# jcasal-homer/HomerHEVC

Hardware: AMD Instinct MI355X
Metric: encoded frames/sec, 1080p & 2160p YUV420 fixed-QP IPPP, 1/2/4/8 MI355X (higher is better)
Workload: dtype int16; 1 GPU; cfg2-1080p-encode; sequences_per_gpu=256, width=1920, height=1080, wfpp_num_threads=17, qp=32, gop=IPPP intra_period=100

## Files before the change

homerhevc_amd/csrc/enc/enc_common.h:

```cpp
#pragma once
#include "enc_prims.h"
#if !defined(__HIPCC__)
#include <stdio.h>
#include <stdlib.h>
#endif

#if !defined(__HIPCC__) && defined(HENC_TRACE_ENABLE)
#include <stdio.h>
extern "C" FILE *henc_trace_file;
#define HENC_TRACE(...) do { if (henc_trace_file) fprintf(henc_trace_file, __VA_ARGS__); } while (0)
#define HENC_TRACE_PW(e, tag)                                                                                                                      \
	do {                                                                                                                                       \
		if (henc_trace_file) {                                                                                                             \
			unsigned a_[3] = {0, 0, 0};                                                                                                \
			for (int c_ = 0; c_ < 3; c_++) {                                                                                           \
				const int n_ = c_ ? 32 : 64;                                                                                       \
				const pred_t *p_ = c_ ? (e).w->pred_c[c_ - 1] : (e).w->pred_y;                                                     \
				for (int y_ = 0; y_ < n_; y_++)                                                                                    \
					for (int x_ = 0; x_ < n_; x_++) a_[c_] += (unsigned)(p_[y_ * n_ + x_] & 0xffff) * (unsigned)(1 + ((x_ + 3 * y_) & 7)); \
			}                                                                                                                          \
			fprintf(henc_trace_file, "PW %s ctu=%d pred=%u,%u,%u\n", tag, (e).ctu->ctu_number, a_[0], a_[1], a_[2]);                   \
		}                                                                                                                                  \
	} while (0)
#else
// ... 324 lines not shown
	HENC_ENC_IN_LDS(e);
	const Geo &gq = e.geo[ni];
	*idx = gq.abs_top_left;
	if (gq.raster_index == 0) return ctu_top_left_of(e);
	if (gq.raster_index < 16) return ctu_top_of(e);
	if ((gq.raster_index & 15) == 0) return ctu_left_of(e);
	return e.ctu;
}

template <class G>
HENC_HD void sync_reference_buffs(const G g, Enc &__restrict__ e, int ni, int src_wnd, int dst_wnd)
{
	HENC_ENC_IN_LDS(e);
	PRIM_T0();
	const Geo &q = e.geo[ni];
	const int16_t *s = dec_ptr(*e.w, src_wnd, COMP_Y) + q.y * DEC_STRIDE_Y + q.x;
	int16_t *d = dec_ptr(*e.w, dst_wnd, COMP_Y) + q.y * DEC_STRIDE_Y + q.x;
	const int n = q.size;
	for (int i = g.tid; i < 2 * n - 1; i += g.n) {
		const int off = i < n ? (n - 1) * DEC_STRIDE_Y + i : (i - n) * DEC_STRIDE_Y + n - 1;
		d[off] = s[off];
	}
	g.sync();
	PRIM_END(PP_SYNC);
}
template <class G>
HENC_HD void sync_reference_buffs_range(const G g, Enc &__restrict__ e, int ni, int src_wnd, int first_dst, int last_dst)
{
	HENC_ENC_IN_LDS(e);
	PRIM_T0();
	const Geo &q = e.geo[ni];
	const int16_t *s = dec_ptr(*e.w, src_wnd, COMP_Y) + q.y * DEC_STRIDE_Y + q.x;
	const int n = q.size, base = q.y * DEC_STRIDE_Y + q.x;
	for (int i0 = g.tid; i0 < 2 * n - 1; i0 += 2 * g.n) {
		const int i1 = i0 + g.n;
		const int off0 = i0 < n ? (n - 1) * DEC_STRIDE_Y + i0 : (i0 - n) * DEC_STRIDE_Y + n - 1;
		const int off1 = i1 < n ? (n - 1) * DEC_STRIDE_Y + i1 : (i1 - n) * DEC_STRIDE_Y + n - 1;
		const bool two = i1 < 2 * n - 1;
		const int16_t v0 = s[off0], v1 = two ? s[off1] : (int16_t)0;
		for (int wnd = first_dst; wnd <= last_dst; wnd++) {
			int16_t *d = dec_ptr(*e.w, wnd, COMP_Y) + base;
			d[off0] = v0;
			if (two) d[off1] = v1;
		}
	}
	g.sync();
	PRIM_END(PP_SYNC);
}
template <class G>
HENC_HD void sync_reference_buffs_chroma(const G g, Enc &__restrict__ e, int ni, int src_wnd, int dst_wnd)
{
	HENC_ENC_IN_LDS(e);
	PRIM_T0();
	const Geo &q = e.geo[ni];
	const int n = q.size_chroma;
	const int16_t *su = dec_ptr(*e.w, src_wnd, COMP_U) + q.yc * DEC_STRIDE_C + q.xc, *sv = dec_ptr(*e.w, src_wnd, COMP_V) + q.yc * DEC_STRIDE_C + q.xc;
	int16_t *du = dec_ptr(*e.w, dst_wnd, COMP_U) + q.yc * DEC_STRIDE_C + q.xc, *dv = dec_ptr(*e.w, dst_wnd, COMP_V) + q.yc * DEC_STRIDE_C + q.xc;
	for (int i = g.tid; i < 2 * n - 1; i += g.n) {
		const int off = i < n ? (n - 1) * DEC_STRIDE_C + i : (i - n) * DEC_STRIDE_C + n - 1;
		const int16_t a = su[off], b = sv[off];
		du[off] = a;
		dv[off] = b;
	}
	g.sync();
	PRIM_END(PP_SYNC);
}
template <class G>
HENC_HD void sync_cu_comp(const G g, Enc &__restrict__ e, int ni, int q_src, int q_dst, int d_src, int d_dst, int comp)
{
	HENC_ENC_IN_LDS(e);
	PRIM_T0();
	const Geo &q = e.geo[ni];
	const int n = comp == COMP_Y ? q.size : q.size_chroma, x = comp == COMP_Y ? q.x : q.xc, y = comp == COMP_Y ? q.y : q.yc;
	const int st = dec_stride(comp), off = comp == COMP_Y ? (q.abs_index << 4) : ((q.abs_index << 4) >> 2);
	const int16_t *ds = dec_ptr(*e.w, d_src, comp) + y * st + x;
	int16_t *dd = dec_ptr(*e.w, d_dst, comp) + y * st + x;
	const int16_t *qs = tq_ptr(*e.w, q_src, comp) + off;
	int16_t *qd = tq_ptr(*e.w, q_dst, comp) + off;
	const int ln = ilog2i(n);
	constexpr int BATCH = 4;
	for (int i0 = g.tid * 4; i0 < n * n; i0 += g.n * 4 * BATCH) {
		S4 a[BATCH], b[BATCH];
#pragma unroll
		for (int u = 0; u < BATCH; u++) {
			const int i = i0 + u * g.n * 4;
			if (i < n * n) {
				a[u] = ld4(ds + (i >> ln) * st + (i & (n - 1)));
				b[u] = ld4(qs + i);
			}
		}
#pragma unroll
		for (int u = 0; u < BATCH; u++) {
			const int i = i0 + u * g.n * 4;
			if (i < n * n) {
				st4(dd + (i >> ln) * st + (i & (n - 1)), a[u]);
				st4(qd + i, b[u]);
			}
		}
	}
	g.sync();
	PRIM_END(PP_SYNC);
}
template <class G>
HENC_HD void sync_cu_chroma_both(const G g, Enc &__restrict__ e, int ni, int q_src, int q_dst, int d_src, int d_dst)
{
	HENC_ENC_IN_LDS(e);
	PRIM_T0();
	const Geo &q = e.geo[ni];
	const int n = q.size_chroma, st = DEC_STRIDE_C, off = (q.abs_index << 4) >> 2, ln = ilog2i(n);
	const int16_t *ds[2], *qs[2];
	int16_t *dd[2], *qd[2];
	for (int c = 0; c < 2; c++) {
		ds[c] = dec_ptr(*e.w, d_src, COMP_U + c) + q.yc * st + q.xc;
		dd[c] = dec_ptr(*e.w, d_dst, COMP_U + c) + q.yc * st + q.xc;
		qs[c] = tq_ptr(*e.w, q_src, COMP_U + c) + off;
		qd[c] = tq_ptr(*e.w, q_dst, COMP_U + c) + off;
	}
	constexpr int BATCH = 2;
	for (int i0 = g.tid * 4; i0 < n * n; i0 += g.n * 4 * BATCH) {
		S4 a[2][BATCH], b[2][BATCH];
#pragma unroll
		for (int u = 0; u < BATCH; u++) {
			const int i = i0 + u * g.n * 4;
			if (i < n * n)
				for (int c = 0; c < 2; c++) {
					a[c][u] = ld4(ds[c] + (i >> ln) * st + (i & (n - 1)));
					b[c][u] = ld4(qs[c] + i);
				}
		}
#pragma unroll
		for (int u = 0; u < BATCH; u++) {
			const int i = i0 + u * g.n * 4;
			if (i < n * n)
				for (int c = 0; c < 2; c++) {
					st4(dd[c] + (i >> ln) * st + (i & (n - 1)), a[c][u]);
					st4(qd[c] + i, b[c][u]);
				}
		}
	}
	g.sync();
	PRIM_END(PP_SYNC);
}
template <class G>
HENC_HD void sync_motion_buffers_luma(const G g, Enc &__restrict__ e, int ni, int q_src, int q_dst, int d_src, int d_dst)
{
	HENC_ENC_IN_LDS(e);
	sync_cu_comp(g, e, ni, q_src, q_dst, d_src, d_dst, COMP_Y);
}
template <class G>
HENC_HD void sync_motion_buffers_chroma(const G g, Enc &__restrict__ e, int ni, int q_src, int q_dst, int d_src, int d_dst)
// ... 62 lines not shown
```

homerhevc_amd/csrc/enc/enc_ctu.h:

```cpp
#pragma once
#include "enc_intra.h"
#include "enc_inter.h"
#include "enc_quad.h"

namespace henc {

template <class G>
HENC_HD void info_buffs_copy(const G g, Enc &__restrict__ e, int depth, int abs_idx, int num, int to_ctu)
{
	HENC_ENC_IN_LDS(e);
	PRIM_T0();
	Work &w = *e.w;
	CtuPublic &c = *e.ctu;
	for (int i = g.tid; i < num; i += g.n) {
		const int k = abs_idx + i;
		if (to_ctu) {
			c.cbf[0][k] = w.cbf_buffs[0][depth][k];
			c.cbf[1][k] = w.cbf_buffs[1][depth][k];
			c.cbf[2][k] = w.cbf_buffs[2][depth][k];
			c.tr_idx[k] = w.tr_idx_buffs[depth][k];
			c.intra_mode[0][k] = w.intra_mode_buffs[0][depth][k];
			c.intra_mode[1][k] = w.intra_mode_buffs[1][depth][k];
		} else {
			const uint8_t v0 = c.cbf[0][k], v1 = c.cbf[1][k], v2 = c.cbf[2][k], v3 = c.tr_idx[k], v4 = c.intra_mode[0][k], v5 = c.intra_mode[1][k];
// ... 738 lines not shown
		blk_copy_to_src(g, e.f->src[comp] + py * ss + px, ss, curr_ptr(w, comp), sz, hh, ww);
	}
	if (c.has_left || c.has_top) {
		for (int comp = 0; comp < 3; comp++) {
			const int sz = comp ? 32 : 64, px = comp ? c.x >> 1 : c.x, py = comp ? c.y >> 1 : c.y;
			const int pw = comp ? S.width >> 1 : S.width, ph = comp ? S.height >> 1 : S.height;
			const int rs = comp ? S.stride_c : S.stride_y, ds = dec_stride(comp);
			int left_copy = 0, top_copy = 0;
			if (c.has_left) left_copy += sz;
			if (c.has_top) top_copy += sz;
			if (c.has_top_right) top_copy += sz;
			if (left_copy > ph - py) left_copy = ph - py;
			if (top_copy > pw - px) top_copy = pw - px;
			const int16_t *src = e.f->rec[comp] + py * rs + px;
			for (int l = 0; l < NWND; l++) {
				int16_t *dst = dec_ptr(w, l, comp);
				for (int i = g.tid; i < 1 + top_copy + left_copy; i += g.n) {
					if (i == 0) {
						if (c.has_left && c.has_top) dst[-ds - 1] = src[-rs - 1];
					} else if (i <= top_copy) dst[-ds + (i - 1)] = src[-rs + (i - 1)];
					else {
						const int j = i - 1 - top_copy;
						dst[j * ds - 1] = src[j * rs - 1];
					}
				}
			}
		}
		g.sync();
	}
	create_partition_neighbours(g, e);
	if (HENC_HELPERS(e)) {
// ... 70 lines not shown
```

homerhevc_amd/csrc/enc/enc_inter.h:

```cpp
#pragma once
#include "enc_common.h"

namespace henc {

#if !defined(__HIPCC__)
template <class G>
HENC_HD void mc_luma_interp(const G g, Enc &__restrict__ e, const int16_t *ref, int rs, int16_t *pred, int ps, int n, int mvx, int mvy)
{
	HENC_ENC_IN_LDS(e);
	const int xf = mvx & 3, yf = mvy & 3;
	const int16_t *src = ref + (mvy >> 2) * rs + (mvx >> 2);
	if (xf == 0) interp_stage<8>(g, src, rs, pred, ps, yf, n, n, 1, 1, 1);
	else if (yf == 0) interp_stage<8>(g, src, rs, pred, ps, xf, n, n, 0, 1, 1);
	else {
		int16_t *tmp = e.mc_tmp_y;
		const int ts = e.mc_tmp_y_stride;
		interp_stage<8>(g, src - 3 * rs, rs, tmp, ts, xf, n, n + 7, 0, 1, 0);
		interp_stage<8>(g, tmp + 3 * ts, ts, pred, ps, yf, n, n, 1, 0, 1);
	}
}
template <class G>
HENC_HD void mc_chroma_interp(const G g, Enc &__restrict__ e, const int16_t *ref, int rs, int16_t *pred, int ps, int n, int mvx, int mvy)
{
	HENC_ENC_IN_LDS(e);
// ... 464 lines not shown
	const int original_depth = e.geo[ni].depth;
	const int pi = (comp == COMP_Y || e.geo[ni].size_chroma != 2) ? ni : e.geo[ni].parent;
	const Geo &q = e.geo[pi];
	const int is_y = comp == COMP_Y;
	const int curr_depth = q.depth, n = is_y ? q.size : q.size_chroma, x = is_y ? q.x : q.xc, y = is_y ? q.y : q.yc;
	const int cs = ctu_stride(comp), ds = dec_stride(comp);
	const int wnd = original_depth + 1 + (part_size_type != PART_2Nx2N);
	const int qp = is_y ? (int)nd.qp : chroma_qp_table((int)nd.qp + e.seq->chroma_qp_offset);
	const int per = qp / 6, rem = qp % 6;
	const double weight = is_y ? 1.0 : e.f->chroma_weight;
	const int off = is_y ? (q.abs_index << 4) : ((q.abs_index << 4) >> 2);
	const pred_t *pred = pred_ptr(w, comp) + y * cs + x;
	const src_t *orig = curr_ptr(w, comp) + y * cs + x;
	int16_t *quant = tq_ptr(w, wnd, comp) + off, *iquant = iq_slot(w, comp, off, e.on_helper) + scratch_off;
	int16_t *const scratch_a = e.scratch_a + scratch_off, *const scratch_b = e.scratch_b + scratch_off;
	int16_t *dec = dec_ptr(w, wnd, comp) + y * ds + x;
	int16_t *rdec = scratch_b;
	tr_forward(g, HENC_FT(e), e.T, orig, cs, pred, cs, scratch_a, scratch_b, n, 0);
	int sum = quantize(g, HENC_FT(e), e.T, scratch_a, iquant, scratch_b, SCAN_DIAG, curr_depth, comp, 0, e.f->slice_type == SLICE_I, e.seq->sign_hiding, n, per, rem);
	nd.inter_cbf[comp] = (sum ? 1 : 0) << (original_depth - depth);
	if (is_y) nd.inter_tr_idx = original_depth - depth;
	uint32_t ssd;
	const bool coded = sum > 0;
	uint32_t raw_zero = 0;
	if (coded) {
		lin_copy_nosync(g, iquant, quant, n * n);
		raw_zero = blk_ssd(g, orig, cs, pred, cs, n);
		if (raw_ssq) *raw_ssq = raw_zero;
		dequantize(g, HENC_FT(e), e.T, iquant, iquant, curr_depth, comp, 0, n, per, rem);
	}
#if defined(HENC_MFMA_TRANSFORM) && !defined(HENC_MFMA_NO_PAIR)
// ... 324 lines not shown
```

homerhevc_amd/csrc/enc/enc_intra.h:

```cpp
#pragma once
#include "enc_common.h"
#include "enc_rdo.h"

namespace henc {

HENC_INLINE int intra_is_filtered(int mode, int inv_depth)
{
	static constexpr int intra_filter[5] = {10, 7, 1, 0, 10};
	const int diff = hmin(habs(mode - HOR_IDX), habs(mode - VER_IDX));
	return (mode != DC_IDX) && (diff > intra_filter[inv_depth - 2]);
}

template <class G>
HENC_HD void node_fill_refs(const G g, Enc &__restrict__ e, int ni, int wnd, int comp, int want_filtered)
{
	HENC_ENC_IN_LDS(e);
	const Geo &q = e.geo[ni];
	const Node &nd = node_of(e, ni);
	const int is_y = comp == COMP_Y;
	const int n = is_y ? q.size : q.size_chroma, x = is_y ? q.x : q.xc, y = is_y ? q.y : q.yc;
	const int pw = is_y ? e.seq->width : e.seq->width >> 1, ph = is_y ? e.seq->height : e.seq->height >> 1;
	const int cx = is_y ? e.ctu_x : e.ctu_x >> 1, cy = is_y ? e.ctu_y : e.ctu_y >> 1;
	const int bl_size = hmin(n, ph - (cy + y + n)), tr_size = hmin(n, pw - (cx + x + n));
	const int st = dec_stride(comp);
	const int16_t *corner = dec_ptr(*e.w, wnd, comp) + (y - 1) * st + (x - 1);
	intra_fill_refs(g, corner, st, n, nd.left_nb, nd.top_nb, nd.left_bottom_nb, nd.top_right_nb, bl_size, tr_size, is_y ? e.w->adi : e.adi_c);
	if (want_filtered) intra_adi_filter(g, e.w->adi, e.w->adi_f, n, e.seq->strong_intra);
}

HENC_INLINE int read_mode_buff(Enc &__restrict__ e, int depth, uint32_t idx, uint16_t *src)
{
	HENC_ENC_IN_LDS(e);
	const int v = e.w->intra_mode_buffs[COMP_Y][depth][idx];
	if (!(v & MODE_TOKEN)) { *src = (uint16_t)v; return v; }
	const int d = v & 7;
	*src = (uint16_t)(0x8000 | (d << 8) | idx);
	return e.w->mode_in[COMP_Y][d][idx];
}
HENC_INLINE void mpm_from_dirs(int left_dir, int top_dir, int *preds)
{
// ... 149 lines not shown

template <class G>
HENC_HD uint32_t encode_intra_tu(const G g, Enc &__restrict__ e, int ni, int depth, int cu_mode, int part_size_type, int *curr_sum)
{
	HENC_ENC_IN_LDS(e);
	const Geo &q = e.geo[ni];
	Node &nd = node_of(e, ni);
	Work &w = *e.w;
	const int curr_depth = q.depth, n = q.size;
	const int scan_mode = find_scan_mode(1, 1, n, cu_mode, 0);
	const int per = nd.qp / 6, rem = nd.qp % 6;
	const int wnd = curr_depth + 1;
	pred_t *pred = w.pred_y + q.y * CTU_STRIDE_Y + q.x;
	const src_t *orig = w.curr_y + q.y * CTU_STRIDE_Y + q.x;
	int16_t *quant = tq_ptr(w, wnd, COMP_Y) + (q.abs_index << 4), *iquant = iq_slot(w, COMP_Y, q.abs_index << 4, e.on_helper);
	int16_t *dec = dec_ptr(w, wnd, COMP_Y) + q.y * DEC_STRIDE_Y + q.x;
	const int inv_depth = CFG_MAX_CU_SHIFT - curr_depth;
	const int filt = intra_is_filtered(cu_mode, inv_depth);
	node_fill_refs(g, e, ni, wnd, COMP_Y, filt);
	intra_predict(g, pred, CTU_STRIDE_Y, filt ? w.adi_f : w.adi, n, cu_mode, 1);
	tr_forward(g, HENC_FT(e), e.T, orig, CTU_STRIDE_Y, pred, CTU_STRIDE_Y, w.pred_aux, w.delta_u, n, cu_mode != REG_DCT);
	const int sum = quantize(g, HENC_FT(e), e.T, w.pred_aux, iquant, w.delta_u, scan_mode, curr_depth, COMP_Y, 1, e.f->slice_type == SLICE_I, e.seq->sign_hiding, n, per, rem);
	*curr_sum = sum;
	const int tr = curr_depth - depth + (part_size_type == PART_NxN);
	nd.sum = (uint32_t)sum;
	nd.intra_cbf[COMP_Y] = (sum ? 1 : 0) << tr;
	nd.intra_tr_idx = tr;
	nd.intra_mode[COMP_Y] = cu_mode;
	if (e.seq->rd_mode == RDM_FULL) set_intra_info_buffs(g, e, curr_depth, ni);
	if (sum) {
		lin_copy_nosync(g, iquant, quant, n * n);
// ... 198 lines not shown
	pred_t *pred = pred_ptr(w, c) + q.yc * CTU_STRIDE_C + q.xc;
	const src_t *orig = curr_ptr(w, c) + q.yc * CTU_STRIDE_C + q.xc;
	node_fill_refs(g, e, curr, NWND - 1, c, 0);
	for (int mi = 0; mi < 5; mi++) sads[mi] = intra_predict_sad(g, pred, CTU_STRIDE_C, orig, CTU_STRIDE_C, e.adi_c, n, cand[mi], 0);
}
template <class G>
HENC_HD int chroma_tu_comp(const G g, Enc &__restrict__ e, int curr, int c, int cu_mode, int scan_mode, int shifts, int per, int rem, int *curr_sum_out)
{
	HENC_ENC_IN_LDS(e);
	Work &w = *e.w;
	const Geo &q = e.geo[curr];
	const int n = q.size_chroma, curr_depth = q.depth, qwnd = NWND - 1, dwnd = NWND - 1;
	pred_t *pred = pred_ptr(w, c) + q.yc * CTU_STRIDE_C + q.xc;
	const src_t *orig = curr_ptr(w, c) + q.yc * CTU_STRIDE_C + q.xc;
	int16_t *quant = tq_ptr(w, qwnd, c) + ((q.abs_index << 4) >> 2), *iquant = iq_slot(w, c, (q.abs_index << 4) >> 2, e.on_helper);
	int16_t *dec = dec_ptr(w, dwnd, c) + q.yc * DEC_STRIDE_C + q.xc;
	node_fill_refs(g, e, curr, dwnd, c, 0);
	intra_predict(g, pred, CTU_STRIDE_C, e.adi_c, n, cu_mode, 0);
	tr_forward(g, HENC_FT(e), e.T, orig, CTU_STRIDE_C, pred, CTU_STRIDE_C, e.scratch_a, e.scratch_b, n, 0);
	const int curr_sum = quantize(g, HENC_FT(e), e.T, e.scratch_a, iquant, e.scratch_b, scan_mode, curr_depth, c, 1, e.f->slice_type == SLICE_I, e.seq->sign_hiding, n, per, rem);
	const int cbfv = ((curr_sum ? 1 : 0) << (shifts & 255)) | ((curr_sum ? 1 : 0) << (shifts >> 8));
	bytes_set(g, &w.cbf_chroma[c - 1][q.abs_index], cbfv, q.num_part);
	uint32_t raw;
	if (curr_sum) {
		lin_copy_nosync(g, iquant, quant, n * n);
		dequantize(g, HENC_FT(e), e.T, iquant, iquant, curr_depth, c, 1, n, per, rem);
		tr_inverse(g, HENC_FT(e), e.T, e.scratch_b, n, iquant, e.scratch_a, n, 0);
		raw = blk_reconst_ssd(g, pred, CTU_STRIDE_C, e.scratch_b, n, orig, CTU_STRIDE_C, dec, DEC_STRIDE_C, n);
	} else {
		lin_zero_nosync(g, quant, n * n);
		raw = blk_reconst_ssd(g, pred, CTU_STRIDE_C, (const int16_t *)nullptr, 0, orig, CTU_STRIDE_C, dec, DEC_STRIDE_C, n);
// ... 212 lines not shown
```

homerhevc_amd/csrc/enc/enc_prims.h:

```cpp
#pragma once
#include "enc_types.h"
#include "../tables_layout.h"

enum { PP_SAD = 0, PP_SSD, PP_BLK, PP_FILLREF, PP_ADIFILT, PP_INTRAPRED, PP_INTERP, PP_TRF, PP_TRI, PP_QUANT, PP_DEQUANT, PP_CAND, PP_SYNC, PP_INFO, PP_CTU_IO, PP_HWAIT, PP_COUNT };
#if defined(__HIPCC__) && defined(HENC_PROFILE)
extern __shared__ __align__(16) unsigned char henc_lds[];
#define HENC_LDS_PROF_OFFSET 43008
#define PRIM_T0() const unsigned long long prim_t0_ = __builtin_amdgcn_s_memtime()
#define PRIM_END(cat) do { if (threadIdx.x == 0) { unsigned long long *pp_ = (unsigned long long *)(henc_lds + HENC_LDS_PROF_OFFSET); pp_[cat] += __builtin_amdgcn_s_memtime() - prim_t0_; pp_[PP_COUNT + (cat)]++; } } while (0)
#else
#define PRIM_T0() do { } while (0)
#define PRIM_END(cat) do { } while (0)
#endif

namespace henc {

HENC_INLINE int ilog2i(int n)
{
	return n <= 1 ? 0 : 32 - __builtin_clz((unsigned)(n - 1));
}
HENC_INLINE void split_rc(int k, int w, int lw, int *r, int *c)
{
	if ((w & (w - 1)) == 0) { *r = k >> lw; *c = k & (w - 1); }
	else { *r = k / w; *c = k - *r * w; }
// ... 4 lines not shown
HENC_INLINE void st4(int16_t *p, const S4 &v) { __builtin_memcpy(p, &v, 8); }
HENC_INLINE S4 ld4(const uint8_t *p)
{
	uint32_t v;
	__builtin_memcpy(&v, p, 4);
	S4 r;
	r.v[0] = (int16_t)(v & 255); r.v[1] = (int16_t)((v >> 8) & 255); r.v[2] = (int16_t)((v >> 16) & 255); r.v[3] = (int16_t)(v >> 24);
	return r;
}

HENC_INLINE void st4(uint8_t *p, const S4 &v)
{
	const uint32_t o = (uint32_t)(v.v[0] & 255) | ((uint32_t)(v.v[1] & 255) << 8) | ((uint32_t)(v.v[2] & 255) << 16) | ((uint32_t)(v.v[3] & 255) << 24);
	__builtin_memcpy(p, &o, 4);
}

template <class G, class S>
HENC_PRIM uint32_t blk_sad(const G g, const S *a, int as, const int16_t *b, int bs, int n)
{
	PRIM_T0();
	const int l = ilog2i(n);
	uint32_t acc = 0;
#pragma unroll 2
	for (int i = g.tid * 4; i < n * n; i += g.n * 4) {
		const int y = i >> l, x = i & (n - 1);
		const S4 va = ld4(a + y * as + x), vb = ld4(b + y * bs + x);
#pragma unroll
		for (int k = 0; k < 4; k++) acc += (uint32_t)habs((int16_t)(va.v[k] - vb.v[k]));
	}
	{ const auto prim_ret_ = g.sum(acc); PRIM_END(PP_SAD); return prim_ret_; }
// ... 143 lines not shown
	PRIM_T0();
	const int l = ilog2i(n);
#pragma unroll 2
	for (int i = g.tid * 4; i < n * n; i += g.n * 4) {
		const int y = i >> l, x = i & (n - 1);
		const S4 vo = ld4(o + y * os + x), vp = ld4(p + y * ps + x);
		S4 vr;
#pragma unroll
		for (int k = 0; k < 4; k++) vr.v[k] = (int16_t)(vo.v[k] - vp.v[k]);
		st4(r + y * rs + x, vr);
	}
	g.sync();
	PRIM_END(PP_BLK);
}

template <class G, class P>
HENC_PRIM void blk_reconst(const G g, const P *p, int ps, const int16_t *res, int rs, int16_t *d, int ds, int n)
{
	PRIM_T0();
	const int l = ilog2i(n);
#pragma unroll 2
	for (int i = g.tid * 4; i < n * n; i += g.n * 4) {
		const int y = i >> l, x = i & (n - 1);
		const S4 vp = ld4(p + y * ps + x);
		S4 vr = {{0, 0, 0, 0}}, vd;
		if (res) vr = ld4(res + y * rs + x);
#pragma unroll
		for (int k = 0; k < 4; k++) vd.v[k] = (int16_t)hclip((int)sat16(vp.v[k] + vr.v[k]), 0, 255);
		st4(d + y * ds + x, vd);
	}
	g.sync();
	PRIM_END(PP_BLK);
}

template <class G, class S, class P>
HENC_PRIM uint32_t blk_reconst_ssd(const G g, const P *p, int ps, const int16_t *res, int rs, const S *o, int os, int16_t *d, int ds, int n)
{
	PRIM_T0();
	const int l = ilog2i(n);
	uint32_t acc = 0;
#pragma unroll 2
	for (int i = g.tid * 4; i < n * n; i += g.n * 4) {
		const int y = i >> l, x = i & (n - 1);
		const S4 vp = ld4(p + y * ps + x), vo = ld4(o + y * os + x);
		S4 vr = {{0, 0, 0, 0}}, vd;
		if (res) vr = ld4(res + y * rs + x);
#pragma unroll
		for (int k = 0; k < 4; k++) {
			vd.v[k] = (int16_t)hclip((int)sat16(vp.v[k] + vr.v[k]), 0, 255);
			const int32_t df = (int16_t)(vo.v[k] - vd.v[k]);
			acc += (uint32_t)(df * df);
		}
		st4(d + y * ds + x, vd);
	}
	const uint32_t s = g.sum(acc);
	g.sync();
	{ const auto prim_ret_ = s; PRIM_END(PP_BLK); return prim_ret_; }
}

template <class G, class P>
HENC_PRIM void blk_copy(const G g, const P *s, int ss, int16_t *d, int ds, int h, int w)
{
	PRIM_T0();
	if ((w & 3) == 0 && (w & (w - 1)) == 0) {
		const int lw = ilog2i(w);
		constexpr int BATCH = 4;
		for (int i0 = g.tid * 4; i0 < h * w; i0 += g.n * 4 * BATCH) {
			S4 v[BATCH];
#pragma unroll
			for (int u = 0; u < BATCH; u++) {
				const int i = i0 + u * g.n * 4;
				if (i < h * w) v[u] = ld4(s + (i >> lw) * ss + (i & (w - 1)));
			}
#pragma unroll
			for (int u = 0; u < BATCH; u++) {
				const int i = i0 + u * g.n * 4;
				if (i < h * w) st4(d + (i >> lw) * ds + (i & (w - 1)), v[u]);
			}
		}
	} else {
		const int lw = ilog2i(w);
		for (int i = g.tid; i < h * w; i += g.n) {
			int y, x;
			split_rc(i, w, lw, &y, &x);
			d[y * ds + x] = s[y * ss + x];
		}
	}
	g.sync();
	PRIM_END(PP_BLK);
}

template <class G>
// ... 93 lines not shown
	PRIM_T0();
	for (int i = g.tid; i < count; i += g.n) d[i] = (uint8_t)v;
	g.sync();
	PRIM_END(PP_BLK);
}

template <class G>
HENC_PRIM void bytes_copy(const G g, const uint8_t *s, uint8_t *d, int count)
{
	PRIM_T0();
	for (int i = g.tid; i < count; i += g.n) d[i] = s[i];
	g.sync();
	PRIM_END(PP_BLK);
}

template <class G>
HENC_PRIM void intra_fill_refs(const G g, const int16_t *corner, int stride, int n, int left, int top, int bottom_left, int top_right,
			     int bl_size, int tr_size, int16_t *adi)
{
	PRIM_T0();
	const int adi_size = 4 * n + 1;
	if (!left && !top) {
		for (int i = g.tid; i < adi_size; i += g.n) adi[i] = 128;
		g.sync();
		{ PRIM_END(PP_FILLREF); return; }
	}
	int pl_ptr = 0, pl_size = 0, pt_ptr = 0, pt_size = 0, first_idx = 0, last_idx = 0;
	if (left) { first_idx = n; last_idx = 2 * n - 1; }
	else { pl_ptr = n; pl_size = n; }
	if (bottom_left) {
		first_idx = n - bl_size;
		if (bl_size != n) { pl_ptr = 0; pl_size = n - bl_size; }
// ... 7 lines not shown
		last_idx = 3 * n;
	} else { pt_ptr = 2 * n + 1; pt_size = n; }
	if (top_right) {
		last_idx = 3 * n + tr_size;
		if (tr_size != n) { pt_ptr = 3 * n + 1 + tr_size; pt_size = n - tr_size; }
	} else {
		if (top) { pt_ptr = 3 * n + 1; pt_size = n; }
		else pt_size += n;
	}
	const bool corner_copy = left && top;
	if (!corner_copy) {
		if (left) { pt_ptr--; pt_size++; }
		else pl_size++;
	}
	auto sample = [&](int k) -> int16_t {
		if (k < n) return corner[(n + 1 + (n - 1 - k)) * stride];
		if (k < 2 * n) return corner[(n - (k - n)) * stride];
		if (k == 2 * n) return corner[0];
		if (k <= 3 * n) return corner[k - 2 * n];
		return corner[1 + n + (k - 3 * n - 1)];
	};
	const int16_t first_sample = sample(first_idx), last_sample = sample(last_idx);
	for (int k = g.tid; k < adi_size; k += g.n) {
		bool avail;
		if (k < n) avail = bottom_left && (n - 1 - k) < bl_size;
		else if (k < 2 * n) avail = left;
		else if (k == 2 * n) avail = corner_copy;
		else if (k <= 3 * n) avail = top;
		else avail = top_right && (k - 3 * n - 1) < tr_size;
		if (k >= pl_ptr && k < pl_ptr + pl_size) adi[k] = first_sample;
		else if (k >= pt_ptr && k < pt_ptr + pt_size) adi[k] = last_sample;
		else if (avail) adi[k] = sample(k);
	}
	g.sync();
	PRIM_END(PP_FILLREF);
// ... 977 lines not shown
```

homerhevc_amd/csrc/enc/enc_quad.h:

```cpp
#pragma once
#include "enc_inter.h"

namespace henc {

#if defined(__HIPCC__) && defined(HENC_MFMA_TRANSFORM) && !defined(HENC_NO_QUAD)
#define HENC_QUAD 1

struct QuadRes {
	uint32_t dist[3];
	int32_t sum[3];
	uint32_t raw[3];
	uint32_t cbf[3];
};
struct QuadScratch {
	union {
		struct {
			uint8_t pred_y[4][64], rec_y[4][64];
			int16_t lv_y[4][64];
			uint8_t pred_c[4][2][16], rec_c[4][2][16];
			int16_t lv_c[4][2][16];
			int16_t wk_lv[256], wk_cf[256], wk_du[256];
		} s8;
		struct {
			uint8_t pred_y[2][256], rec_y[2][256];
// ... 333 lines not shown
template <int CU>
__device__ __forceinline__ void quad_commit(const WaveGrp g, Enc &__restrict__ e, int ni, int depth, int cons_slot, int cons_kind, int wnd_slot, int wnd_kind, int last_pred, int coded_any)
{
	HENC_ENC_IN_LDS(e);
	Work &w = *e.w;
	const Geo &q = e.geo[ni];
	const Node &nd = node_of(e, ni);
	CtuPublic &c = *e.ctu;
	QuadScratch &qs = quad_scratch(e);
	const S4 zero = {{0, 0, 0, 0}};
	constexpr int NC = CU / 2, YL = CU * CU / 4, CL = 2 * NC * NC / 4;
	auto luma = [&](int l) {
		const int r = l / (CU / 4), c0 = (l % (CU / 4)) * 4;
		if (cons_kind) {
			st4(tq_ptr(w, 0, COMP_Y) + (q.abs_index << 4) + l * 4, cons_kind == 1 ? ld4(quad_lv_y<CU>(qs, cons_slot) + l * 4) : zero);
			st4(dec_ptr(w, 0, COMP_Y) + (q.y + r) * DEC_STRIDE_Y + q.x + c0, ld4((cons_kind == 1 ? quad_rec_y<CU>(qs, cons_slot) : quad_pred_y<CU>(qs, cons_slot)) + r * CU + c0));
		}
		if (wnd_kind) {
			st4(tq_ptr(w, depth + 1, COMP_Y) + (q.abs_index << 4) + l * 4, wnd_kind == 1 ? ld4(quad_lv_y<CU>(qs, wnd_slot) + l * 4) : zero);
			st4(dec_ptr(w, depth + 1, COMP_Y) + (q.y + r) * DEC_STRIDE_Y + q.x + c0, ld4((wnd_kind == 1 ? quad_rec_y<CU>(qs, wnd_slot) : quad_pred_y<CU>(qs, wnd_slot)) + r * CU + c0));
		}
		if (last_pred >= 0) *(uint32_t *)(w.pred_y + (q.y + r) * 64 + q.x + c0) = *(const uint32_t *)(quad_pred_y<CU>(qs, last_pred) + r * CU + c0);
	};
	auto chroma = [&](int l) {
		const int p = l / (NC * NC / 4), j = l % (NC * NC / 4), r = j / (NC / 4), c0 = (j % (NC / 4)) * 4;
		if (cons_kind) {
			st4(tq_ptr(w, 0, COMP_U + p) + ((q.abs_index << 4) >> 2) + j * 4, cons_kind == 1 ? ld4(quad_lv_c<CU>(qs, cons_slot, p) + j * 4) : zero);
			st4(dec_ptr(w, 0, COMP_U + p) + (q.yc + r) * DEC_STRIDE_C + q.xc + c0, ld4((cons_kind == 1 ? quad_rec_c<CU>(qs, cons_slot, p) : quad_pred_c<CU>(qs, cons_slot, p)) + r * NC + c0));
		}
		if (wnd_kind) {
			st4(tq_ptr(w, depth + 1, COMP_U + p) + ((q.abs_index << 4) >> 2) + j * 4, wnd_kind == 1 ? ld4(quad_lv_c<CU>(qs, wnd_slot, p) + j * 4) : zero);
			st4(dec_ptr(w, depth + 1, COMP_U + p) + (q.yc + r) * DEC_STRIDE_C + q.xc + c0, ld4((wnd_kind == 1 ? quad_rec_c<CU>(qs, wnd_slot, p) : quad_pred_c<CU>(qs, wnd_slot, p)) + r * NC + c0));
		}
		if (last_pred >= 0) *(uint32_t *)(w.pred_c[p] + (q.yc + r) * 32 + q.xc + c0) = *(const uint32_t *)(quad_pred_c<CU>(qs, last_pred, p) + r * NC + c0);
	};
	auto info = [&](int u) {
		const int k = q.abs_index + u;
		if (cons_kind) {
			const QuadRes &cr = qs.res[cons_slot];
			c.cbf[0][k] = cons_kind == 1 ? (uint8_t)cr.cbf[0] : (uint8_t)0;
			c.cbf[1][k] = cons_kind == 1 ? (uint8_t)cr.cbf[1] : (uint8_t)0;
			c.cbf[2][k] = cons_kind == 1 ? (uint8_t)cr.cbf[2] : (uint8_t)0;
			c.tr_idx[k] = 0;
			c.intra_mode[0][k] = w.intra_mode_buffs[0][depth][k];
			c.intra_mode[1][k] = w.intra_mode_buffs[1][depth][k];
		}
		if (wnd_kind) {
// ... 137 lines not shown
```

homerhevc_amd/csrc/enc/enc_types.h:

```cpp
#pragma once
#include "enc_platform.h"

namespace henc {

enum { COMP_Y = 0, COMP_U = 1, COMP_V = 2, COMP_CHR = 1 };
enum { PM_INTER = 0, PM_INTRA = 1 };
enum { PART_2Nx2N = 0, PART_NxN = 3 };
enum { SLICE_B = 0, SLICE_P = 1, SLICE_I = 2 };
enum { RDM_DIST_ONLY = 0, RDM_FULL = 1, RDM_FAST = 2 };
enum { ME_PEL = 1, ME_HALF = 2, ME_QUARTER = 4 };
enum { PLANAR_IDX = 0, DC_IDX = 1, HOR_IDX = 10, VER_IDX = 26, DM_CHROMA_IDX = 36, REG_DCT = 65535 };
enum { SCAN_ZIGZAG = 0, SCAN_HOR = 1, SCAN_VER = 2, SCAN_DIAG = 3 };

constexpr int NPART = 256;
constexpr int NNODES = 341;
constexpr int NDEPTH = 5;
constexpr int NWND = 7;
constexpr uint32_t MAX_COST = 0xffffffffu / 8;

constexpr int MAX_SEARCH_LOGS = 192, MAX_RATIO_CMP = 96;
constexpr int POST_MAX_ROWS = 128;
constexpr int HENC_MAX_STEPS = 192;
constexpr int MODE_TOKEN = 0x80;

constexpr int SEARCH_RANGE_X = 128, SEARCH_RANGE_Y = 64;

constexpr int DEC_STRIDE_Y = 144, DEC_ROWS_Y = 130, DEC_ORG_Y = 1 * DEC_STRIDE_Y + 8;
constexpr int DEC_STRIDE_C = 80, DEC_ROWS_C = 66, DEC_ORG_C = 1 * DEC_STRIDE_C + 8;
constexpr int CTU_STRIDE_Y = 64, CTU_STRIDE_C = 32;

struct MV {
	int32_t x, y;
};

struct Geo {
	int32_t list_index, depth, abs_index, size, size_chroma, x, y, xc, yc, num_part, raster_index;
	int32_t abs_left, abs_left_bottom, abs_top, abs_top_right, abs_top_left;
	int32_t parent;
	int32_t child[4];
};

struct MV16 {
	int16_t x, y;
	HENC_INLINE operator MV() const { MV m = {x, y}; return m; }
// ... 88 lines not shown
	double avg_dist, lambda, sqrt_lambda, chroma_weight;
	double sao_lambda[3];
	const int16_t *src[3];
	const int16_t *ref[3];
	int16_t *rec[3];
	const uint8_t *sub_y, *sub_c[2];
	RcFrame rc;
};

struct MvCandList {
	int32_t num;
	MV mv[5];
	int32_t ref_idx[5];
};

struct WorkSlow {
	int16_t rdec_y[64 * 64], rdec_c[2][32 * 32];
	int16_t tq_y[NWND][64 * 64], tq_c[NWND][2][32 * 32];
	int16_t dec_y[NWND][DEC_ROWS_Y * DEC_STRIDE_Y], dec_c[NWND][2][DEC_ROWS_C * DEC_STRIDE_C];
};

#if defined(__HIPCC__)
typedef uint8_t pred_t;
#else
typedef int16_t pred_t;
#endif
#if defined(__HIPCC__)
typedef uint8_t src_t;
constexpr int TU_SCRATCH = 32 * 32;
#else
typedef int16_t src_t;
constexpr int TU_SCRATCH = 64 * 64;
#endif

struct EntScratch {
// ... 42 lines not shown
	HENC_GLOBAL_PTR(WorkSlow) slow;
	int32_t thread_seen_intra;
#if !defined(__HIPCC__)
	struct WorkRd *rd_store;
#endif
};
struct WorkRd {
	uint8_t rd_pred_depth[NPART], rd_part_size[NPART], rd_pred_mode[NPART], rd_luma_modes[NPART];
	uint8_t rd_ctx_work[RD_CTX_BYTES];
	EntScratch rd_ent;
	alignas(8) unsigned char rd_views[512];
};

HENC_INLINE int16_t *wnd_y(int16_t *base) { return base; }

HENC_INLINE int16_t *dec_ptr(Work &w, int wnd, int comp)
{
	return (int16_t *)(comp == COMP_Y ? w.slow->dec_y[wnd] + DEC_ORG_Y : w.slow->dec_c[wnd][comp - 1] + DEC_ORG_C);
}
HENC_INLINE int dec_stride(int comp) { return comp == COMP_Y ? DEC_STRIDE_Y : DEC_STRIDE_C; }
HENC_INLINE int ctu_stride(int comp) { return comp == COMP_Y ? CTU_STRIDE_Y : CTU_STRIDE_C; }
HENC_INLINE int16_t *tq_ptr(Work &w, int wnd, int comp) { return (int16_t *)(comp == COMP_Y ? w.slow->tq_y[wnd] : w.slow->tq_c[wnd][comp - 1]); }
HENC_INLINE src_t *curr_ptr(Work &w, int comp) { return comp == COMP_Y ? w.curr_y : w.curr_c[comp - 1]; }
HENC_INLINE pred_t *pred_ptr(Work &w, int comp) { return comp == COMP_Y ? w.pred_y : w.pred_c[comp - 1]; }
HENC_INLINE int16_t *rdec_ptr(Work &w, int comp) { return (int16_t *)(comp == COMP_Y ? w.slow->rdec_y : w.slow->rdec_c[comp - 1]); }
HENC_INLINE int16_t *iq_slot(Work &w, int comp, int off, int on_helper)
{
#if defined(__HIPCC__)
	(void)off; (void)comp;
	return on_helper ? w.iq_c[on_helper - 1] : w.iq_y;
#else
	(void)on_helper;
	return (comp == COMP_Y ? w.iq_y : w.iq_c[comp - 1]) + off;
#endif
}

}
```

Measured before the change: 467.9 frames/s.

## Store decoded reconstruction windows as bytes with cache-line aligned rows

Switches the per-worker decoded and rdec windows from int16 to uint8 on the GPU build and widens the row strides and origins so each row and the CTU's 64/32 columns plus the left neighbour sit within one 128-byte line. Copy, reconstruct and reference-fill primitives are templated on the destination type, with packed 4-byte load/store helpers. This halves the global memory footprint and traffic of the reconstruction window copies between RD windows. The risk is narrowing when int16 sources are packed to bytes; that is only correct if reconstructed samples are already clipped to 8 bits.

```diff
diff --git a/homerhevc_amd/csrc/enc/enc_common.h b/homerhevc_amd/csrc/enc/enc_common.h
--- a/homerhevc_amd/csrc/enc/enc_common.h
+++ b/homerhevc_amd/csrc/enc/enc_common.h
@@ -362,8 +362,8 @@
 	HENC_ENC_IN_LDS(e);
 	PRIM_T0();
 	const Geo &q = e.geo[ni];
-	const int16_t *s = dec_ptr(*e.w, src_wnd, COMP_Y) + q.y * DEC_STRIDE_Y + q.x;
-	int16_t *d = dec_ptr(*e.w, dst_wnd, COMP_Y) + q.y * DEC_STRIDE_Y + q.x;
+	const dec_t *s = dec_ptr(*e.w, src_wnd, COMP_Y) + q.y * DEC_STRIDE_Y + q.x;
+	dec_t *d = dec_ptr(*e.w, dst_wnd, COMP_Y) + q.y * DEC_STRIDE_Y + q.x;
 	const int n = q.size;
 	for (int i = g.tid; i < 2 * n - 1; i += g.n) {
 		const int off = i < n ? (n - 1) * DEC_STRIDE_Y + i : (i - n) * DEC_STRIDE_Y + n - 1;
@@ -378,16 +378,16 @@
 	HENC_ENC_IN_LDS(e);
 	PRIM_T0();
 	const Geo &q = e.geo[ni];
-	const int16_t *s = dec_ptr(*e.w, src_wnd, COMP_Y) + q.y * DEC_STRIDE_Y + q.x;
+	const dec_t *s = dec_ptr(*e.w, src_wnd, COMP_Y) + q.y * DEC_STRIDE_Y + q.x;
 	const int n = q.size, base = q.y * DEC_STRIDE_Y + q.x;
 	for (int i0 = g.tid; i0 < 2 * n - 1; i0 += 2 * g.n) {
 		const int i1 = i0 + g.n;
 		const int off0 = i0 < n ? (n - 1) * DEC_STRIDE_Y + i0 : (i0 - n) * DEC_STRIDE_Y + n - 1;
 		const int off1 = i1 < n ? (n - 1) * DEC_STRIDE_Y + i1 : (i1 - n) * DEC_STRIDE_Y + n - 1;
 		const bool two = i1 < 2 * n - 1;
-		const int16_t v0 = s[off0], v1 = two ? s[off1] : (int16_t)0;
+		const dec_t v0 = s[off0], v1 = two ? s[off1] : (dec_t)0;
 		for (int wnd = first_dst; wnd <= last_dst; wnd++) {
-			int16_t *d = dec_ptr(*e.w, wnd, COMP_Y) + base;
+			dec_t *d = dec_ptr(*e.w, wnd, COMP_Y) + base;
 			d[off0] = v0;
 			if (two) d[off1] = v1;
 		}
@@ -402,11 +402,11 @@
 	PRIM_T0();
 	const Geo &q = e.geo[ni];
 	const int n = q.size_chroma;
-	const int16_t *su = dec_ptr(*e.w, src_wnd, COMP_U) + q.yc * DEC_STRIDE_C + q.xc, *sv = dec_ptr(*e.w, src_wnd, COMP_V) + q.yc * DEC_STRIDE_C + q.xc;
-	int16_t *du = dec_ptr(*e.w, dst_wnd, COMP_U) + q.yc * DEC_STRIDE_C + q.xc, *dv = dec_ptr(*e.w, dst_wnd, COMP_V) + q.yc * DEC_STRIDE_C + q.xc;
+	const dec_t *su = dec_ptr(*e.w, src_wnd, COMP_U) + q.yc * DEC_STRIDE_C + q.xc, *sv = dec_ptr(*e.w, src_wnd, COMP_V) + q.yc * DEC_STRIDE_C + q.xc;
+	dec_t *du = dec_ptr(*e.w, dst_wnd, COMP_U) + q.yc * DEC_STRIDE_C + q.xc, *dv = dec_ptr(*e.w, dst_wnd, COMP_V) + q.yc * DEC_STRIDE_C + q.xc;
 	for (int i = g.tid; i < 2 * n - 1; i += g.n) {
 		const int off = i < n ? (n - 1) * DEC_STRIDE_C + i : (i - n) * DEC_STRIDE_C + n - 1;
-		const int16_t a = su[off], b = sv[off];
+		const dec_t a = su[off], b = sv[off];
 		du[off] = a;
 		dv[off] = b;
 	}
@@ -421,19 +421,20 @@
 	const Geo &q = e.geo[ni];
 	const int n = comp == COMP_Y ? q.size : q.size_chroma, x = comp == COMP_Y ? q.x : q.xc, y = comp == COMP_Y ? q.y : q.yc;
 	const int st = dec_stride(comp), off = comp == COMP_Y ? (q.abs_index << 4) : ((q.abs_index << 4) >> 2);
-	const int16_t *ds = dec_ptr(*e.w, d_src, comp) + y * st + x;
-	int16_t *dd = dec_ptr(*e.w, d_dst, comp) + y * st + x;
+	const dec_t *ds = dec_ptr(*e.w, d_src, comp) + y * st + x;
+	dec_t *dd = dec_ptr(*e.w, d_dst, comp) + y * st + x;
 	const int16_t *qs = tq_ptr(*e.w, q_src, comp) + off;
 	int16_t *qd = tq_ptr(*e.w, q_dst, comp) + off;
 	const int ln = ilog2i(n);
 	constexpr int BATCH = 4;
 	for (int i0 = g.tid * 4; i0 < n * n; i0 += g.n * 4 * BATCH) {
-		S4 a[BATCH], b[BATCH];
+		Quad<dec_t>::T a[BATCH];
+		S4 b[BATCH];
 #pragma unroll
 		for (int u = 0; u < BATCH; u++) {
 			const int i = i0 + u * g.n * 4;
 			if (i < n * n) {
-				a[u] = ld4(ds + (i >> ln) * st + (i & (n - 1)));
+				ld4q(ds + (i >> ln) * st + (i & (n - 1)), a[u]);
 				b[u] = ld4(qs + i);
 			}
 		}
@@ -441,7 +442,7 @@
 		for (int u = 0; u < BATCH; u++) {
 			const int i = i0 + u * g.n * 4;
 			if (i < n * n) {
-				st4(dd + (i >> ln) * st + (i & (n - 1)), a[u]);
+				st4q(dd + (i >> ln) * st + (i & (n - 1)), a[u]);
 				st4(qd + i, b[u]);
 			}
 		}
@@ -456,8 +457,10 @@
 	PRIM_T0();
 	const Geo &q = e.geo[ni];
 	const int n = q.size_chroma, st = DEC_STRIDE_C, off = (q.abs_index << 4) >> 2, ln = ilog2i(n);
-	const int16_t *ds[2], *qs[2];
-	int16_t *dd[2], *qd[2];
+	const dec_t *ds[2];
+	dec_t *dd[2];
+	const int16_t *qs[2];
+	int16_t *qd[2];
 	for (int c = 0; c < 2; c++) {
 		ds[c] = dec_ptr(*e.w, d_src, COMP_U + c) + q.yc * st + q.xc;
 		dd[c] = dec_ptr(*e.w, d_dst, COMP_U + c) + q.yc * st + q.xc;
@@ -466,13 +469,14 @@
 	}
 	constexpr int BATCH = 2;
 	for (int i0 = g.tid * 4; i0 < n * n; i0 += g.n * 4 * BATCH) {
-		S4 a[2][BATCH], b[2][BATCH];
+		Quad<dec_t>::T a[2][BATCH];
+		S4 b[2][BATCH];
 #pragma unroll
 		for (int u = 0; u < BATCH; u++) {
 			const int i = i0 + u * g.n * 4;
 			if (i < n * n)
 				for (int c = 0; c < 2; c++) {
-					a[c][u] = ld4(ds[c] + (i >> ln) * st + (i & (n - 1)));
+					ld4q(ds[c] + (i >> ln) * st + (i & (n - 1)), a[c][u]);
 					b[c][u] = ld4(qs[c] + i);
 				}
 		}
@@ -481,7 +485,7 @@
 			const int i = i0 + u * g.n * 4;
 			if (i < n * n)
 				for (int c = 0; c < 2; c++) {
-					st4(dd[c] + (i >> ln) * st + (i & (n - 1)), a[c][u]);
+					st4q(dd[c] + (i >> ln) * st + (i & (n - 1)), a[c][u]);
 					st4(qd[c] + i, b[c][u]);
 				}
 		}
diff --git a/homerhevc_amd/csrc/enc/enc_ctu.h b/homerhevc_amd/csrc/enc/enc_ctu.h
--- a/homerhevc_amd/csrc/enc/enc_ctu.h
+++ b/homerhevc_amd/csrc/enc/enc_ctu.h
@@ -776,7 +776,7 @@
 			if (top_copy > pw - px) top_copy = pw - px;
 			const int16_t *src = e.f->rec[comp] + py * rs + px;
 			for (int l = 0; l < NWND; l++) {
-				int16_t *dst = dec_ptr(w, l, comp);
+				dec_t *dst = dec_ptr(w, l, comp);
 				for (int i = g.tid; i < 1 + top_copy + left_copy; i += g.n) {
 					if (i == 0) {
 						if (c.has_left && c.has_top) dst[-ds - 1] = src[-rs - 1];
diff --git a/homerhevc_amd/csrc/enc/enc_inter.h b/homerhevc_amd/csrc/enc/enc_inter.h
--- a/homerhevc_amd/csrc/enc/enc_inter.h
+++ b/homerhevc_amd/csrc/enc/enc_inter.h
@@ -502,7 +502,7 @@
 	const src_t *orig = curr_ptr(w, comp) + y * cs + x;
 	int16_t *quant = tq_ptr(w, wnd, comp) + off, *iquant = iq_slot(w, comp, off, e.on_helper) + scratch_off;
 	int16_t *const scratch_a = e.scratch_a + scratch_off, *const scratch_b = e.scratch_b + scratch_off;
-	int16_t *dec = dec_ptr(w, wnd, comp) + y * ds + x;
+	dec_t *dec = dec_ptr(w, wnd, comp) + y * ds + x;
 	int16_t *rdec = scratch_b;
 	tr_forward(g, HENC_FT(e), e.T, orig, cs, pred, cs, scratch_a, scratch_b, n, 0);
 	int sum = quantize(g, HENC_FT(e), e.T, scratch_a, iquant, scratch_b, SCAN_DIAG, curr_depth, comp, 0, e.f->slice_type == SLICE_I, e.seq->sign_hiding, n, per, rem);
diff --git a/homerhevc_amd/csrc/enc/enc_intra.h b/homerhevc_amd/csrc/enc/enc_intra.h
--- a/homerhevc_amd/csrc/enc/enc_intra.h
+++ b/homerhevc_amd/csrc/enc/enc_intra.h
@@ -23,7 +23,7 @@
 	const int cx = is_y ? e.ctu_x : e.ctu_x >> 1, cy = is_y ? e.ctu_y : e.ctu_y >> 1;
 	const int bl_size = hmin(n, ph - (cy + y + n)), tr_size = hmin(n, pw - (cx + x + n));
 	const int st = dec_stride(comp);
-	const int16_t *corner = dec_ptr(*e.w, wnd, comp) + (y - 1) * st + (x - 1);
+	const dec_t *corner = dec_ptr(*e.w, wnd, comp) + (y - 1) * st + (x - 1);
 	intra_fill_refs(g, corner, st, n, nd.left_nb, nd.top_nb, nd.left_bottom_nb, nd.top_right_nb, bl_size, tr_size, is_y ? e.w->adi : e.adi_c);
 	if (want_filtered) intra_adi_filter(g, e.w->adi, e.w->adi_f, n, e.seq->strong_intra);
 }
@@ -203,7 +203,7 @@
 	pred_t *pred = w.pred_y + q.y * CTU_STRIDE_Y + q.x;
 	const src_t *orig = w.curr_y + q.y * CTU_STRIDE_Y + q.x;
 	int16_t *quant = tq_ptr(w, wnd, COMP_Y) + (q.abs_index << 4), *iquant = iq_slot(w, COMP_Y, q.abs_index << 4, e.on_helper);
-	int16_t *dec = dec_ptr(w, wnd, COMP_Y) + q.y * DEC_STRIDE_Y + q.x;
+	dec_t *dec = dec_ptr(w, wnd, COMP_Y) + q.y * DEC_STRIDE_Y + q.x;
 	const int inv_depth = CFG_MAX_CU_SHIFT - curr_depth;
 	const int filt = intra_is_filtered(cu_mode, inv_depth);
 	node_fill_refs(g, e, ni, wnd, COMP_Y, filt);
@@ -432,7 +432,7 @@
 	pred_t *pred = pred_ptr(w, c) + q.yc * CTU_STRIDE_C + q.xc;
 	const src_t *orig = curr_ptr(w, c) + q.yc * CTU_STRIDE_C + q.xc;
 	int16_t *quant = tq_ptr(w, qwnd, c) + ((q.abs_index << 4) >> 2), *iquant = iq_slot(w, c, (q.abs_index << 4) >> 2, e.on_helper);
-	int16_t *dec = dec_ptr(w, dwnd, c) + q.yc * DEC_STRIDE_C + q.xc;
+	dec_t *dec = dec_ptr(w, dwnd, c) + q.yc * DEC_STRIDE_C + q.xc;
 	node_fill_refs(g, e, curr, dwnd, c, 0);
 	intra_predict(g, pred, CTU_STRIDE_C, e.adi_c, n, cu_mode, 0);
 	tr_forward(g, HENC_FT(e), e.T, orig, CTU_STRIDE_C, pred, CTU_STRIDE_C, e.scratch_a, e.scratch_b, n, 0);
diff --git a/homerhevc_amd/csrc/enc/enc_prims.h b/homerhevc_amd/csrc/enc/enc_prims.h
--- a/homerhevc_amd/csrc/enc/enc_prims.h
+++ b/homerhevc_amd/csrc/enc/enc_prims.h
@@ -42,6 +42,17 @@
 	const uint32_t o = (uint32_t)(v.v[0] & 255) | ((uint32_t)(v.v[1] & 255) << 8) | ((uint32_t)(v.v[2] & 255) << 16) | ((uint32_t)(v.v[3] & 255) << 24);
 	__builtin_memcpy(p, &o, 4);
 }
+template <class D> struct Quad { typedef S4 T; };
+template <> struct Quad<uint8_t> { typedef uint32_t T; };
+HENC_INLINE void ld4q(const uint8_t *p, uint32_t &v) { __builtin_memcpy(&v, p, 4); }
+HENC_INLINE void ld4q(const int16_t *p, uint32_t &v)
+{
+	const S4 s = ld4(p);
+	v = (uint32_t)(s.v[0] & 255) | ((uint32_t)(s.v[1] & 255) << 8) | ((uint32_t)(s.v[2] & 255) << 16) | ((uint32_t)(s.v[3] & 255) << 24);
+}
+template <class S> HENC_INLINE void ld4q(const S *p, S4 &v) { v = ld4(p); }
+HENC_INLINE void st4q(uint8_t *p, uint32_t v) { __builtin_memcpy(p, &v, 4); }
+HENC_INLINE void st4q(int16_t *p, const S4 &v) { st4(p, v); }
 
 template <class G, class S>
 HENC_PRIM uint32_t blk_sad(const G g, const S *a, int as, const int16_t *b, int bs, int n)
@@ -215,8 +226,8 @@
 	PRIM_END(PP_BLK);
 }
 
-template <class G, class P>
-HENC_PRIM void blk_reconst(const G g, const P *p, int ps, const int16_t *res, int rs, int16_t *d, int ds, int n)
+template <class G, class P, class D>
+HENC_PRIM void blk_reconst(const G g, const P *p, int ps, const int16_t *res, int rs, D *d, int ds, int n)
 {
 	PRIM_T0();
 	const int l = ilog2i(n);
@@ -234,8 +245,8 @@
 	PRIM_END(PP_BLK);
 }
 
-template <class G, class S, class P>
-HENC_PRIM uint32_t blk_reconst_ssd(const G g, const P *p, int ps, const int16_t *res, int rs, const S *o, int os, int16_t *d, int ds, int n)
+template <class G, class S, class P, class D>
+HENC_PRIM uint32_t blk_reconst_ssd(const G g, const P *p, int ps, const int16_t *res, int rs, const S *o, int os, D *d, int ds, int n)
 {
 	PRIM_T0();
 	const int l = ilog2i(n);
@@ -259,24 +270,24 @@
 	{ const auto prim_ret_ = s; PRIM_END(PP_BLK); return prim_ret_; }
 }
 
-template <class G, class P>
-HENC_PRIM void blk_copy(const G g, const P *s, int ss, int16_t *d, int ds, int h, int w)
+template <class G, class P, class D>
+HENC_PRIM void blk_copy(const G g, const P *s, int ss, D *d, int ds, int h, int w)
 {
 	PRIM_T0();
 	if ((w & 3) == 0 && (w & (w - 1)) == 0) {
 		const int lw = ilog2i(w);
 		constexpr int BATCH = 4;
 		for (int i0 = g.tid * 4; i0 < h * w; i0 += g.n * 4 * BATCH) {
-			S4 v[BATCH];
+			typename Quad<D>::T v[BATCH];
 #pragma unroll
 			for (int u = 0; u < BATCH; u++) {
 				const int i = i0 + u * g.n * 4;
-				if (i < h * w) v[u] = ld4(s + (i >> lw) * ss + (i & (w - 1)));
+				if (i < h * w) ld4q(s + (i >> lw) * ss + (i & (w - 1)), v[u]);
 			}
 #pragma unroll
 			for (int u = 0; u < BATCH; u++) {
 				const int i = i0 + u * g.n * 4;
-				if (i < h * w) st4(d + (i >> lw) * ds + (i & (w - 1)), v[u]);
+				if (i < h * w) st4q(d + (i >> lw) * ds + (i & (w - 1)), v[u]);
 			}
 		}
 	} else {
@@ -400,8 +411,8 @@
 	PRIM_END(PP_BLK);
 }
 
-template <class G>
-HENC_PRIM void intra_fill_refs(const G g, const int16_t *corner, int stride, int n, int left, int top, int bottom_left, int top_right,
+template <class G, class D>
+HENC_PRIM void intra_fill_refs(const G g, const D *corner, int stride, int n, int left, int top, int bottom_left, int top_right,
 			     int bl_size, int tr_size, int16_t *adi)
 {
 	PRIM_T0();
@@ -439,11 +450,11 @@
 		else pl_size++;
 	}
 	auto sample = [&](int k) -> int16_t {
-		if (k < n) return corner[(n + 1 + (n - 1 - k)) * stride];
-		if (k < 2 * n) return corner[(n - (k - n)) * stride];
-		if (k == 2 * n) return corner[0];
-		if (k <= 3 * n) return corner[k - 2 * n];
-		return corner[1 + n + (k - 3 * n - 1)];
+		if (k < n) return (int16_t)corner[(n + 1 + (n - 1 - k)) * stride];
+		if (k < 2 * n) return (int16_t)corner[(n - (k - n)) * stride];
+		if (k == 2 * n) return (int16_t)corner[0];
+		if (k <= 3 * n) return (int16_t)corner[k - 2 * n];
+		return (int16_t)corner[1 + n + (k - 3 * n - 1)];
 	};
 	const int16_t first_sample = sample(first_idx), last_sample = sample(last_idx);
 	for (int k = g.tid; k < adi_size; k += g.n) {
diff --git a/homerhevc_amd/csrc/enc/enc_quad.h b/homerhevc_amd/csrc/enc/enc_quad.h
--- a/homerhevc_amd/csrc/enc/enc_quad.h
+++ b/homerhevc_amd/csrc/enc/enc_quad.h
@@ -371,11 +371,11 @@
 		const int r = l / (CU / 4), c0 = (l % (CU / 4)) * 4;
 		if (cons_kind) {
 			st4(tq_ptr(w, 0, COMP_Y) + (q.abs_index << 4) + l * 4, cons_kind == 1 ? ld4(quad_lv_y<CU>(qs, cons_slot) + l * 4) : zero);
-			st4(dec_ptr(w, 0, COMP_Y) + (q.y + r) * DEC_STRIDE_Y + q.x + c0, ld4((cons_kind == 1 ? quad_rec_y<CU>(qs, cons_slot) : quad_pred_y<CU>(qs, cons_slot)) + r * CU + c0));
+			st4q(dec_ptr(w, 0, COMP_Y) + (q.y + r) * DEC_STRIDE_Y + q.x + c0, *(const uint32_t *)((cons_kind == 1 ? quad_rec_y<CU>(qs, cons_slot) : quad_pred_y<CU>(qs, cons_slot)) + r * CU + c0));
 		}
 		if (wnd_kind) {
 			st4(tq_ptr(w, depth + 1, COMP_Y) + (q.abs_index << 4) + l * 4, wnd_kind == 1 ? ld4(quad_lv_y<CU>(qs, wnd_slot) + l * 4) : zero);
-			st4(dec_ptr(w, depth + 1, COMP_Y) + (q.y + r) * DEC_STRIDE_Y + q.x + c0, ld4((wnd_kind == 1 ? quad_rec_y<CU>(qs, wnd_slot) : quad_pred_y<CU>(qs, wnd_slot)) + r * CU + c0));
+			st4q(dec_ptr(w, depth + 1, COMP_Y) + (q.y + r) * DEC_STRIDE_Y + q.x + c0, *(const uint32_t *)((wnd_kind == 1 ? quad_rec_y<CU>(qs, wnd_slot) : quad_pred_y<CU>(qs, wnd_slot)) + r * CU + c0));
 		}
 		if (last_pred >= 0) *(uint32_t *)(w.pred_y + (q.y + r) * 64 + q.x + c0) = *(const uint32_t *)(quad_pred_y<CU>(qs, last_pred) + r * CU + c0);
 	};
@@ -383,11 +383,11 @@
 		const int p = l / (NC * NC / 4), j = l % (NC * NC / 4), r = j / (NC / 4), c0 = (j % (NC / 4)) * 4;
 		if (cons_kind) {
 			st4(tq_ptr(w, 0, COMP_U + p) + ((q.abs_index << 4) >> 2) + j * 4, cons_kind == 1 ? ld4(quad_lv_c<CU>(qs, cons_slot, p) + j * 4) : zero);
-			st4(dec_ptr(w, 0, COMP_U + p) + (q.yc + r) * DEC_STRIDE_C + q.xc + c0, ld4((cons_kind == 1 ? quad_rec_c<CU>(qs, cons_slot, p) : quad_pred_c<CU>(qs, cons_slot, p)) + r * NC + c0));
+			st4q(dec_ptr(w, 0, COMP_U + p) + (q.yc + r) * DEC_STRIDE_C + q.xc + c0, *(const uint32_t *)((cons_kind == 1 ? quad_rec_c<CU>(qs, cons_slot, p) : quad_pred_c<CU>(qs, cons_slot, p)) + r * NC + c0));
 		}
 		if (wnd_kind) {
 			st4(tq_ptr(w, depth + 1, COMP_U + p) + ((q.abs_index << 4) >> 2) + j * 4, wnd_kind == 1 ? ld4(quad_lv_c<CU>(qs, wnd_slot, p) + j * 4) : zero);
-			st4(dec_ptr(w, depth + 1, COMP_U + p) + (q.yc + r) * DEC_STRIDE_C + q.xc + c0, ld4((wnd_kind == 1 ? quad_rec_c<CU>(qs, wnd_slot, p) : quad_pred_c<CU>(qs, wnd_slot, p)) + r * NC + c0));
+			st4q(dec_ptr(w, depth + 1, COMP_U + p) + (q.yc + r) * DEC_STRIDE_C + q.xc + c0, *(const uint32_t *)((wnd_kind == 1 ? quad_rec_c<CU>(qs, wnd_slot, p) : quad_pred_c<CU>(qs, wnd_slot, p)) + r * NC + c0));
 		}
 		if (last_pred >= 0) *(uint32_t *)(w.pred_c[p] + (q.yc + r) * 32 + q.xc + c0) = *(const uint32_t *)(quad_pred_c<CU>(qs, last_pred, p) + r * NC + c0);
 	};
diff --git a/homerhevc_amd/csrc/enc/enc_types.h b/homerhevc_amd/csrc/enc/enc_types.h
--- a/homerhevc_amd/csrc/enc/enc_types.h
+++ b/homerhevc_amd/csrc/enc/enc_types.h
@@ -1,4 +1,5 @@
 #pragma once
+#include <stddef.h>
 #include "enc_platform.h"
 
 namespace henc {
@@ -25,9 +26,16 @@
 
 constexpr int SEARCH_RANGE_X = 128, SEARCH_RANGE_Y = 64;
 
-constexpr int DEC_STRIDE_Y = 144, DEC_ROWS_Y = 130, DEC_ORG_Y = 1 * DEC_STRIDE_Y + 8;
-constexpr int DEC_STRIDE_C = 80, DEC_ROWS_C = 66, DEC_ORG_C = 1 * DEC_STRIDE_C + 8;
+constexpr int DEC_STRIDE_Y = 256, DEC_ROWS_Y = 130, DEC_ORG_Y = 1 * DEC_STRIDE_Y + 64;
+constexpr int DEC_STRIDE_C = 128, DEC_ROWS_C = 66, DEC_ORG_C = 1 * DEC_STRIDE_C + 32;
 constexpr int CTU_STRIDE_Y = 64, CTU_STRIDE_C = 32;
+constexpr int DEC_LINE = 128;
+static_assert(DEC_STRIDE_Y % DEC_LINE == 0 && DEC_STRIDE_C % DEC_LINE == 0, "decoded window rows start on a line");
+static_assert(DEC_ORG_Y / DEC_STRIDE_Y == 1 && DEC_ORG_C / DEC_STRIDE_C == 1, "row -1 precedes the origin");
+static_assert(DEC_ORG_Y % DEC_STRIDE_Y >= 1 && DEC_ORG_Y % DEC_LINE >= 1 && DEC_ORG_Y % DEC_LINE + 64 <= DEC_LINE, "luma: column -1 and the CTU's 64 columns in one line");
+static_assert(DEC_ORG_C % DEC_STRIDE_C >= 1 && DEC_ORG_C % DEC_LINE >= 1 && DEC_ORG_C % DEC_LINE + 32 <= DEC_LINE, "chroma: column -1 and the CTU's 32 columns in one line");
+static_assert(DEC_ORG_Y % DEC_STRIDE_Y + 128 <= DEC_STRIDE_Y && DEC_ORG_C % DEC_STRIDE_C + 64 <= DEC_STRIDE_C, "the area right of the origin fits a row");
+static_assert(DEC_ROWS_Y >= 1 + 128 && DEC_ROWS_C >= 1 + 64, "the area below the origin fits the window");
 
 struct MV {
 	int32_t x, y;
@@ -146,11 +154,20 @@
 	int32_t ref_idx[5];
 };
 
+#if defined(__HIPCC__) || defined(HENC_DEC_BYTES)
+typedef uint8_t dec_t;
+#else
+typedef int16_t dec_t;
+#endif
+
 struct WorkSlow {
-	int16_t rdec_y[64 * 64], rdec_c[2][32 * 32];
+	dec_t rdec_y[64 * 64], rdec_c[2][32 * 32];
 	int16_t tq_y[NWND][64 * 64], tq_c[NWND][2][32 * 32];
-	int16_t dec_y[NWND][DEC_ROWS_Y * DEC_STRIDE_Y], dec_c[NWND][2][DEC_ROWS_C * DEC_STRIDE_C];
-};
+	dec_t dec_y[NWND][DEC_ROWS_Y * DEC_STRIDE_Y], dec_c[NWND][2][DEC_ROWS_C * DEC_STRIDE_C];
+};
+static_assert(offsetof(WorkSlow, dec_y) % DEC_LINE == 0 && offsetof(WorkSlow, dec_c) % DEC_LINE == 0 && sizeof(WorkSlow) % DEC_LINE == 0,
+	      "every worker's windows start on a line");
+static_assert(sizeof(dec_t) != 1 || sizeof(WorkSlow) == 443392, "WorkSlow with byte windows");
 
 #if defined(__HIPCC__)
 typedef uint8_t pred_t;
@@ -223,16 +240,16 @@
 
 HENC_INLINE int16_t *wnd_y(int16_t *base) { return base; }
 
-HENC_INLINE int16_t *dec_ptr(Work &w, int wnd, int comp)
+HENC_INLINE dec_t *dec_ptr(Work &w, int wnd, int comp)
 {
-	return (int16_t *)(comp == COMP_Y ? w.slow->dec_y[wnd] + DEC_ORG_Y : w.slow->dec_c[wnd][comp - 1] + DEC_ORG_C);
+	return (dec_t *)(comp == COMP_Y ? w.slow->dec_y[wnd] + DEC_ORG_Y : w.slow->dec_c[wnd][comp - 1] + DEC_ORG_C);
 }
 HENC_INLINE int dec_stride(int comp) { return comp == COMP_Y ? DEC_STRIDE_Y : DEC_STRIDE_C; }
 HENC_INLINE int ctu_stride(int comp) { return comp == COMP_Y ? CTU_STRIDE_Y : CTU_STRIDE_C; }
 HENC_INLINE int16_t *tq_ptr(Work &w, int wnd, int comp) { return (int16_t *)(comp == COMP_Y ? w.slow->tq_y[wnd] : w.slow->tq_c[wnd][comp - 1]); }
 HENC_INLINE src_t *curr_ptr(Work &w, int comp) { return comp == COMP_Y ? w.curr_y : w.curr_c[comp - 1]; }
 HENC_INLINE pred_t *pred_ptr(Work &w, int comp) { return comp == COMP_Y ? w.pred_y : w.pred_c[comp - 1]; }
-HENC_INLINE int16_t *rdec_ptr(Work &w, int comp) { return (int16_t *)(comp == COMP_Y ? w.slow->rdec_y : w.slow->rdec_c[comp - 1]); }
+HENC_INLINE dec_t *rdec_ptr(Work &w, int comp) { return (dec_t *)(comp == COMP_Y ? w.slow->rdec_y : w.slow->rdec_c[comp - 1]); }
 HENC_INLINE int16_t *iq_slot(Work &w, int comp, int off, int on_helper)
 {
 #if defined(__HIPCC__)
```

New measurement: 472.6 frames/s, median of 6. About the same (+1.0%).
